# airlift/aircompressor

Hardware: AMD Instinct MI355X
Metric: GiB/s decompressed throughput (Zstd+LZ4) at 1/2/4/8 GPUs; % of HBM3E roofline (higher is better)
Workload: dtype u8; 1 GPU; lz4_decompress, 262144 x 65536 B LZ4 blocks per GPU (BASELINE configs[1]), fragments data ratio=0.50, LZ4 ratio 1.817, batched C-ABI launch, HBM-resident; blocks_per_gpu=262144, block_bytes=65536, distinct_blocks=4096, parallelism=block-sharded x1, no collective, decoder=rings (chosen on the device: 0 of 16384 16-block groups mixed), twopass_fallback_blocks=-1

## Files before the change

### aircompressor_amd/csrc/achip_rings.h

```cpp
#pragma once
#include "achip_device.h"

namespace achip {


template <int GS, int IN_RING, int OUT_RING, int GPL = 1, int PHASED = 0>
struct Rings {
    static constexpr int CHUNK = GS * 16 * GPL;
    static constexpr int LDS_REACH = OUT_RING - CHUNK - 16;
    static_assert((IN_RING & (IN_RING - 1)) == 0 && (OUT_RING & (OUT_RING - 1)) == 0, "rings are powers of two");
    static_assert(IN_RING >= 2 * CHUNK && OUT_RING >= 4 * CHUNK, "ring too small for the chunk size");
    static_assert(!PHASED || (IN_RING >= 4 * CHUNK && GS == 4 && GPL == 1), "the phased form keeps two chunks of input ahead");
    static constexpr bool PH_REFILL = PHASED != 0, PH_FLUSH = false;

    uint8_t* inRing;
    uint8_t* outRing;
    const uint8_t* inAligned;
    uint8_t* outAligned;
    int32_t inBase, outBase;
    int32_t inEndV;
    int32_t inLoadedV;
    int32_t flushedV;
    u32x4 pending[GPL];
    int g;
    uint8_t* stage;

    static constexpr bool UNIFIED = GS == 4 && GPL == 1;

#if !defined(__HIPCC__) && defined(HOSTEMU_RINGS_LOCKSTEP)
    __device__ __forceinline__ void order() const { if (GS > 1) hostemu::group_sync(GS, __FILE__, __LINE__); }
    __device__ __forceinline__ void enter() const { if (GS > 1) hostemu::group_sync(GS, __FILE__, __LINE__); }
#elif !defined(__HIPCC__) && defined(HOSTEMU_RINGS_ORDER_ONLY)
    __device__ __forceinline__ void order() const { if (GS > 1) hostemu::group_sync(GS, __FILE__, __LINE__); }
    __device__ __forceinline__ void enter() const {}
#else
    __device__ __forceinline__ void order() const { wave_mem_order(); }
    __device__ __forceinline__ void enter() const {}
#endif

    __device__ __forceinline__ void init(uint8_t* ldsIn, uint8_t* ldsOut, const uint8_t* in, int32_t inLimit, uint8_t* out, int lane, uint8_t* ldsStage = nullptr)
    {
        inRing = ldsIn;
        outRing = ldsOut;
        stage = ldsStage;
        inBase = (int32_t)((uintptr_t)in & 15);
        outBase = (int32_t)((uintptr_t)out & 15);
        inAligned = in - inBase;
        outAligned = out - outBase;
        inEndV = inLimit + inBase;
        inLoadedV = 0;
        flushedV = 0;
        g = lane;
        if (PHASED) {
            request_pending(16 * g);
        }
        else {
#pragma unroll
            for (int q = 0; q < GPL; q++) {
                pending[q] = fetch_granule(16 * (g + GS * q));
            }
        }
    }

    __device__ __forceinline__ void request_pending(int32_t v) { pending[0] = fetch_granule(v); }
    __device__ __forceinline__ u32x4 take_pending(int32_t) { return pending[0]; }

    __device__ __forceinline__ void reset_input(const uint8_t* in, int32_t inLimit)
    {
        enter();
        inBase = (int32_t)((uintptr_t)in & 15);
        inAligned = in - inBase;
        inEndV = inLimit + inBase;
        inLoadedV = 0;
        order();
#pragma unroll
        for (int q = 0; q < GPL; q++) {
            pending[q] = fetch_granule(16 * (g + GS * q));
        }
    }

    __device__ __forceinline__ u32x4 fetch_granule(int32_t v) const
    {
        u32x4 d = {0, 0, 0, 0};
        if (v >= inBase && v + 16 <= inEndV) {
            d = ld16_global(inAligned + v);
        }
        else if (v + 16 > inBase && v < inEndV) {
            uint32_t w[4] = {0, 0, 0, 0};
#pragma unroll 1
            for (int i = 0; i < 16; i++) {
                const int32_t p = v + i;
                if (p >= inBase && p < inEndV) {
                    w[i >> 2] |= (uint32_t)inAligned[p] << (8 * (i & 3));
                }
            }
            d = u32x4{w[0], w[1], w[2], w[3]};
        }
        return d;
    }

    __device__ __forceinline__ void refill()
    {
        if (PHASED) {
            const int32_t v = inLoadedV + 16 * g;
            *(u32x4*)(inRing + (v & (IN_RING - 1))) = take_pending(v);
            request_pending(v + CHUNK);
            inLoadedV += CHUNK;
            return;
        }
#pragma unroll
        for (int q = 0; q < GPL; q++) {
            const int32_t v = inLoadedV + 16 * (g + GS * q);
            *(u32x4*)(inRing + (v & (IN_RING - 1))) = pending[q];
            pending[q] = fetch_granule(v + CHUNK);
        }
        inLoadedV += CHUNK;
    }
    __device__ __forceinline__ void ensure_input(int32_t pos, int32_t need)
    {
        enter();
        const int32_t want = pos + inBase + need;
        if (want > inLoadedV && inLoadedV < inEndV) {
            do {
                refill();
            } while (want > inLoadedV && inLoadedV < inEndV);
        }
        order();
    }
    __device__ __forceinline__ uint32_t in_u8(int32_t pos) const { return inRing[(pos + inBase) & (IN_RING - 1)]; }

    __device__ __forceinline__ void memory_phase(int32_t ip, int32_t op)
    {
        if (PHASED) {
            enter();
            if (PH_REFILL && inLoadedV - (ip + inBase) <= IN_RING - CHUNK && inLoadedV < inEndV) {
                refill();
            }
            order();
            if (PH_FLUSH) {
                flush_complete(op);
            }
        }
    }

    template <int RING>
    static __device__ __forceinline__ uint32_t ring_ld4(const uint8_t* ring, int32_t pv)
    {
        const int32_t a = pv & ~3;
        const uint32_t lo = *(const uint32_t*)(ring + (a & (RING - 1)));
        const uint32_t hi = *(const uint32_t*)(ring + ((a + 4) & (RING - 1)));
        return alignbyte_u32(hi, lo, (uint32_t)(pv & 3));
    }


    template <int SRC_RING>
    __device__ __forceinline__ void copy_dwords(const uint8_t* src, int32_t sV, int32_t dV, int32_t c)
    {
        copy_dwords_rt(src, SRC_RING - 1, sV, dV, c);
    }

    __device__ __forceinline__ void put4(int32_t dV, uint32_t w, int32_t cnt)
    {
        if (cnt > 0) outRing[dV & (OUT_RING - 1)] = (uint8_t)w;
        if (cnt > 1) outRing[(dV + 1) & (OUT_RING - 1)] = (uint8_t)(w >> 8);
        if (cnt > 2) outRing[(dV + 2) & (OUT_RING - 1)] = (uint8_t)(w >> 16);
        if (cnt > 3) outRing[(dV + 3) & (OUT_RING - 1)] = (uint8_t)(w >> 24);
    }
    template <int SRC_RING>
    __device__ __forceinline__ void copy_small(const uint8_t* src, int32_t sV, int32_t dV, int32_t n)
    {
        const uint32_t w = ring_ld4<SRC_RING>(src, sV + 4 * g);
        enter();
        put4(dV + 4 * g, w, n - 4 * g);
    }

    static __device__ __forceinline__ uint32_t ring_ld4_rt(const uint8_t* ring, int32_t mask, int32_t pv)
    {
        const int32_t a = pv & ~3;
        const uint32_t lo = *(const uint32_t*)(ring + (a & mask));
        const uint32_t hi = *(const uint32_t*)(ring + ((a + 4) & mask));
        return alignbyte_u32(hi, lo, (uint32_t)(pv & 3));
    }
    __device__ __forceinline__ void copy_dwords_rt(const uint8_t* src, int32_t mask, int32_t sV, int32_t dV, int32_t c)
    {
        int32_t head = (4 - (dV & 3)) & 3;
        head = head < c ? head : c;
        constexpr int ITER = CHUNK / (4 * GS);
        uint32_t w[ITER];
#pragma unroll
        for (int q = 0; q < ITER; q++) {
            w[q] = ring_ld4_rt(src, mask, sV + head + 4 * (g + GS * q));
        }
        uint32_t hb[3] = {0, 0, 0};
#pragma unroll
        for (int k = 0; k < 3; k++) {
            if ((k & (GS - 1)) == g && k < head) {
                hb[k] = src[(sV + k) & mask];
            }
        }
        enter();
#pragma unroll
        for (int q = 0; q < ITER; q++) {
            *(uint32_t*)(outRing + ((dV + head + 4 * (g + GS * q)) & (OUT_RING - 1))) = w[q];
        }
#pragma unroll
        for (int k = 0; k < 3; k++) {
            if ((k & (GS - 1)) == g && k < head) {
                outRing[(dV + k) & (OUT_RING - 1)] = (uint8_t)hb[k];
            }
        }
    }

    __device__ __forceinline__ void out_put(int32_t pos, uint32_t byte) { outRing[(pos + outBase) & (OUT_RING - 1)] = (uint8_t)byte; }
    __device__ __forceinline__ uint32_t out_get(int32_t pos) const { return outRing[(pos + outBase) & (OUT_RING - 1)]; }

    __device__ __forceinline__ void flush_complete(int32_t op)
    {
        enter();
        const int32_t opV = op + outBase;
        order();
        while (flushedV + CHUNK <= opV) {
#pragma unroll
            for (int q = 0; q < GPL; q++) {
                const int32_t v = flushedV + 16 * (g + GS * q);
                if (v >= outBase) {
                    *(u32x4*)(outAligned + v) = *(const u32x4*)(outRing + (v & (OUT_RING - 1)));
                }
                else if (v + 16 > outBase) {
                    for (int32_t p = outBase; p < v + 16; p++) {
                        outAligned[p] = outRing[p & (OUT_RING - 1)];
                    }
                }
            }
            flushedV += CHUNK;
        }
        order();
    }
    __device__ __forceinline__ void flush_all(int32_t op)
    {
        flush_complete(op);
        const int32_t opV = op + outBase;
#pragma unroll
        for (int q = 0; q < GPL; q++) {
            const int32_t v = flushedV + 16 * (g + GS * q);
            if (v < opV) {
                if (v >= outBase && v + 16 <= opV) {
                    *(u32x4*)(outAligned + v) = *(const u32x4*)(outRing + (v & (OUT_RING - 1)));
                }
                else {
                    const int32_t lo = v > outBase ? v : outBase;
                    const int32_t hi = v + 16 < opV ? v + 16 : opV;
                    for (int32_t p = lo; p < hi; p++) {
                        outAligned[p] = outRing[p & (OUT_RING - 1)];
                    }
                }
            }
        }
        flushedV = opV & ~15;
        order();
    }

    __device__ __forceinline__ void fill(int32_t op, uint32_t value, int32_t n)
    {
        enter();
        while (n > 0) {
            const int32_t c = n < CHUNK ? n : CHUNK;
            for (int32_t k = g; k < c; k += GS) {
                out_put(op + k, value);
            }
            op += c;
            n -= c;
            flush_complete(op);
        }
    }

    __device__ __forceinline__ void copy_literals(int32_t ip, int32_t op, int32_t n)
    {
        enter();
        if (UNIFIED && n > 4 * GS) {
            while (n > 0) {
                const int32_t c = n < CHUNK ? n : CHUNK;
                ensure_input(ip, c);
                copy_dwords<IN_RING>(inRing, ip + inBase, op + outBase, c);
                ip += c;
                op += c;
                n -= c;
                if (!PH_FLUSH || n > 0) {
                    flush_complete(op);
                }
            }
            return;
        }
        if (n <= 4 * GS) {
            ensure_input(ip, n);
            copy_small<IN_RING>(inRing, ip + inBase, op + outBase, n);
            if (!PH_FLUSH) {
                flush_complete(op + n);
            }
            return;
        }
        while (n > 0) {
            const int32_t c = n < CHUNK ? n : CHUNK;
            ensure_input(ip, c);
            if (c <= (GS > 4 ? GS : 4)) {
                for (int32_t k = g; k < c; k += GS) {
                    out_put(op + k, in_u8(ip + k));
                }
            }
            else {
                copy_dwords<IN_RING>(inRing, ip + inBase, op + outBase, c);
            }
            ip += c;
            op += c;
            n -= c;
            flush_complete(op);
        }
    }

    __device__ __forceinline__ void copy_match(int32_t op, int32_t offset, int32_t n)
    {
        enter();
        if (UNIFIED && !(n <= 4 * GS && offset >= n)) {
            if (stage != nullptr) {
                int32_t dist = offset;
                while (n > 0) {
                    int32_t c = n < CHUNK ? n : CHUNK;
                    c = c < dist ? c : dist;
                    order();
                    if (dist <= LDS_REACH) {
                        copy_dwords<OUT_RING>(outRing, op + outBase - dist, op + outBase, c);
                    }
                    else {
                        if (PH_FLUSH && op + outBase - dist + CHUNK > flushedV) {
                            flush_complete(op);
                            order();
                        }
                        *(u32x4*)(stage + 16 * g) = ld16(outAligned + outBase + (op - dist) + 16 * g);
                        order();
                        copy_dwords<CHUNK>(stage, 0, op + outBase, c);
                    }
                    op += c;
                    n -= c;
                    if (dist < CHUNK) {
                        dist += dist;
                    }
                    if (!PH_FLUSH || n > 0) {
                        flush_complete(op);
                    }
                }
                return;
            }
        }
        if (n <= 4 * GS && offset >= n) {
            order();
            if (offset <= LDS_REACH) {
                copy_small<OUT_RING>(outRing, op + outBase - offset, op + outBase, n);
            }
            else {
                if (PH_FLUSH && op + outBase - offset + 4 * GS > flushedV) {
                    flush_complete(op);
                    order();
                }
                put4(op + outBase + 4 * g, ld4(outAligned + outBase + (op - offset) + 4 * g), n - 4 * g);
            }
            if (!PH_FLUSH) {
                flush_complete(op + n);
            }
            return;
        }
        int32_t c0 = op;
        while (n > 0) {
            const int32_t c = n < CHUNK ? n : CHUNK;
            order();
            if (offset <= LDS_REACH) {
                if (offset >= c && c <= (GS > 4 ? GS : 4)) {
                    for (int32_t j = g; j < c; j += GS) {
                        out_put(c0 + j, out_get(c0 - offset + j));
                    }
                }
                else if (offset >= c) {
                    copy_dwords<OUT_RING>(outRing, c0 + outBase - offset, c0 + outBase, c);
                }
                else {
                    const uint32_t inv = offset == 1 ? 0u : (0xFFFFFFFFu / (uint32_t)offset + 1u);
                    for (int32_t j = g; j < c; j += GS) {
                        const uint32_t q = offset == 1 ? (uint32_t)j : __umulhi((uint32_t)j, inv);
                        out_put(c0 + j, out_get(c0 - offset + (j - (int32_t)q * offset)));
                    }
                }
            }
            else {
                const uint8_t* src = outAligned + outBase + (c0 - offset);
                if (c <= (GS > 4 ? GS : 4)) {
                    for (int32_t j = g; j < c; j += GS) {
                        out_put(c0 + j, src[j]);
                    }
                }
                else {
                    const int32_t dV = c0 + outBase;
                    const int32_t head = (4 - (dV & 3)) & 3;
                    const int32_t nd = (c - head) >> 2;
                    const int32_t t0 = head + 4 * nd;
                    for (int32_t k = g; k < head; k += GS) {
                        outRing[(dV + k) & (OUT_RING - 1)] = src[k];
                    }
                    for (int32_t j = g; j < nd; j += GS) {
                        *(uint32_t*)(outRing + ((dV + head + 4 * j) & (OUT_RING - 1))) = ld4(src + head + 4 * j);
                    }
                    for (int32_t k = t0 + g; k < c; k += GS) {
                        outRing[(dV + k) & (OUT_RING - 1)] = src[k];
                    }
                }
            }
            c0 += c;
            n -= c;
            flush_complete(c0);
        }
    }
};

}
```

### aircompressor_amd/csrc/lz4_decode_body.h

```cpp
#pragma once
#include "achip_rings.h"

namespace achip {

template <int GS, int IN_RING, int OUT_RING, int GPL, int PHASED = 0>
__device__ __forceinline__ void lz4_block_decode(Rings<GS, IN_RING, OUT_RING, GPL, PHASED>& R, const uint8_t* __restrict__ in, int32_t inLimit, int32_t outLimit, int32_t& stOut,
                                                 int32_t& eoOut, int32_t& opOut)
{
    int32_t st = 0;
    int32_t eo = 0;
    int32_t ip = 0;
    int32_t op = 0;

#define LZ4_FAIL(detail, off)                          \
    {                                                  \
        st = mk_status(ACHIP_CLASS_MALFORMED, detail); \
        eo = (int32_t)(off);                           \
        break;                                         \
    }

    if (inLimit == 0) {
        st = mk_status(ACHIP_CLASS_MALFORMED, ACHIP_D_LZ4_INPUT_EMPTY);
    }
    else if (outLimit == 0) {
        if (!(inLimit == 1 && in[0] == 0)) {
            st = mk_status(ACHIP_CLASS_OUTPUT_TOO_SMALL, ACHIP_D_LZ4_EMPTY_OUTPUT);
        }
    }
    else {
        const int32_t fastOutLimit = outLimit - 8;
        R.ensure_input(ip, 4);
        uint32_t t4 = R.template ring_ld4<IN_RING>(R.inRing, ip + R.inBase);
        while (ip < inLimit) {
            const int32_t token = (int32_t)(t4 & 0xFF);
            ip++;

            int32_t lit = token >> 4;
            if (lit == 0xF) {
                if (ip >= inLimit) LZ4_FAIL(ACHIP_D_LZ4_MALFORMED, ip);
                int32_t v = (int32_t)((t4 >> 8) & 0xFF);
                ip++;
                lit = (int32_t)((uint32_t)lit + (uint32_t)v);
                while (v == 255 && ip < inLimit - 15) {
                    R.ensure_input(ip, 1);
                    v = (int32_t)R.in_u8(ip++);
                    lit = (int32_t)((uint32_t)lit + (uint32_t)v);
                }
            }
            if (lit < 0) LZ4_FAIL(ACHIP_D_LZ4_MALFORMED, ip);

            const int64_t litEnd = (int64_t)ip + lit;
            const int64_t litOutLimit = (int64_t)op + lit;
            if (litOutLimit > fastOutLimit - 4 || litEnd > inLimit - 8) {
                if (litOutLimit > outLimit) LZ4_FAIL(ACHIP_D_LZ4_LAST_LITERAL_OUTSIDE, ip);
                if (litEnd != inLimit) LZ4_FAIL(ACHIP_D_LZ4_INPUT_NOT_CONSUMED, ip);
                R.copy_literals(ip, op, lit);
                op += lit;
                break;
            }

            uint32_t o4 = 0;
            const bool early = lit + 3 <= Rings<GS, IN_RING, OUT_RING, GPL, PHASED>::CHUNK;
            if (early) {
                R.ensure_input(ip, lit + 3);
                o4 = R.template ring_ld4<IN_RING>(R.inRing, (int32_t)litEnd + R.inBase);
            }
            R.copy_literals(ip, op, lit);
            op += lit;
            ip = (int32_t)litEnd;
            R.memory_phase(ip, op);

            if (!early) {
                R.ensure_input(ip, 3);
                o4 = R.template ring_ld4<IN_RING>(R.inRing, ip + R.inBase);
            }
            const int32_t offset = (int32_t)(o4 & 0xFFFF);
            ip += 2;
            if (offset == 0 || offset > op) LZ4_FAIL(ACHIP_D_LZ4_OFFSET_OUTSIDE, ip);

            int32_t ml = token & 0xF;
            if (ml == 0xF) {
                if (ip > inLimit - 5) LZ4_FAIL(ACHIP_D_LZ4_MALFORMED, ip);
                int32_t v = (int32_t)((o4 >> 16) & 0xFF);
                ip++;
                ml = (int32_t)((uint32_t)ml + (uint32_t)v);
                bool bad = false;
                while (v == 255) {
                    if (ip > inLimit - 5) {
                        bad = true;
                        break;
                    }
                    R.ensure_input(ip, 1);
                    v = (int32_t)R.in_u8(ip++);
                    ml = (int32_t)((uint32_t)ml + (uint32_t)v);
                }
                if (bad) LZ4_FAIL(ACHIP_D_LZ4_MALFORMED, ip);
            }
            ml = (int32_t)((uint32_t)ml + 4u);
            if (ml < 0) LZ4_FAIL(ACHIP_D_LZ4_MALFORMED, ip);

            const int64_t matchOutLimit = (int64_t)op + ml;
            if (matchOutLimit > fastOutLimit - 4 && matchOutLimit > outLimit - 5) {
                LZ4_FAIL(ACHIP_D_LZ4_LAST_5_LITERALS, ip);
            }
            R.ensure_input(ip, 4);
            t4 = R.template ring_ld4<IN_RING>(R.inRing, ip + R.inBase);
            R.copy_match(op, offset, ml);
            op = (int32_t)matchOutLimit;
        }
        R.flush_all(op);
    }
#undef LZ4_FAIL
    stOut = st;
    eoOut = eo;
    opOut = op;
}

}
```

Before: 2012 GiB/s.

## Streamline 4-lane ring copies with dword-aligned moves and single-step flushes

In the unified decoder path, copy_dwords_rt is replaced by a fixed four-dword-per-lane move aligned to the destination. It merges the partial head dword with the existing ring contents and caps each move at CHUNK minus the misalignment. The flush loop becomes a single-step flush per move, and literals already in the input ring skip the ensure_input check. LZ4 bounds checks in the narrow configuration use precomputed unsigned thresholds. The aim is to cut per-sequence branching and loop overhead. The cost is that correctness now depends on the cap and flush-step invariants, such as flushing at most one chunk per move.

```diff
diff --git a/aircompressor_amd/csrc/achip_rings.h b/aircompressor_amd/csrc/achip_rings.h
--- a/aircompressor_amd/csrc/achip_rings.h
+++ b/aircompressor_amd/csrc/achip_rings.h
@@ -153,6 +153,8 @@
     }
 
 
+    static __device__ __forceinline__ int32_t move_cap(int32_t dV) { return UNIFIED ? CHUNK - (dV & 3) : CHUNK; }
+
     template <int SRC_RING>
     __device__ __forceinline__ void copy_dwords(const uint8_t* src, int32_t sV, int32_t dV, int32_t c)
     {
@@ -183,6 +185,25 @@
     }
     __device__ __forceinline__ void copy_dwords_rt(const uint8_t* src, int32_t mask, int32_t sV, int32_t dV, int32_t c)
     {
+        if (UNIFIED) {
+            const int32_t k = dV & 3;
+            const int32_t s0 = sV - k + 4 * g;
+            const int32_t dI = dV - k + 4 * g;
+            uint32_t w[4];
+#pragma unroll
+            for (int q = 0; q < 4; q++) {
+                w[q] = ring_ld4_rt(src, mask, s0 + 16 * q);
+            }
+            const uint32_t prev = *(const uint32_t*)(outRing + (dI & (OUT_RING - 1)));
+            const uint32_t mine = 0xFFFFFFFFu << (8 * (g == 0 ? k : 0));
+            w[0] = (w[0] & mine) | (prev & ~mine);
+            enter();
+#pragma unroll
+            for (int q = 0; q < 4; q++) {
+                *(uint32_t*)(outRing + ((dI + 16 * q) & (OUT_RING - 1))) = w[q];
+            }
+            return;
+        }
         int32_t head = (4 - (dV & 3)) & 3;
         head = head < c ? head : c;
         constexpr int ITER = CHUNK / (4 * GS);
@@ -230,6 +251,29 @@
                     for (int32_t p = outBase; p < v + 16; p++) {
                         outAligned[p] = outRing[p & (OUT_RING - 1)];
                     }
+                }
+            }
+            flushedV += CHUNK;
+        }
+        order();
+    }
+    __device__ __forceinline__ void flush_step(int32_t op)
+    {
+        if (!UNIFIED) {
+            flush_complete(op);
+            return;
+        }
+        enter();
+        const int32_t opV = op + outBase;
+        order();
+        if (flushedV + CHUNK <= opV) {
+            const int32_t v = flushedV + 16 * g;
+            if (flushedV != 0 || v >= outBase) {
+                *(u32x4*)(outAligned + v) = *(const u32x4*)(outRing + (v & (OUT_RING - 1)));
+            }
+            else if (v + 16 > outBase) {
+                for (int32_t p = outBase; p < v + 16; p++) {
+                    outAligned[p] = outRing[p & (OUT_RING - 1)];
                 }
             }
             flushedV += CHUNK;
@@ -279,14 +323,15 @@
         enter();
         if (UNIFIED && n > 4 * GS) {
             while (n > 0) {
-                const int32_t c = n < CHUNK ? n : CHUNK;
+                const int32_t cap = move_cap(op + outBase);
+                const int32_t c = n < cap ? n : cap;
                 ensure_input(ip, c);
                 copy_dwords<IN_RING>(inRing, ip + inBase, op + outBase, c);
                 ip += c;
                 op += c;
                 n -= c;
                 if (!PH_FLUSH || n > 0) {
-                    flush_complete(op);
+                    flush_step(op);
                 }
             }
             return;
@@ -295,7 +340,7 @@
             ensure_input(ip, n);
             copy_small<IN_RING>(inRing, ip + inBase, op + outBase, n);
             if (!PH_FLUSH) {
-                flush_complete(op + n);
+                flush_step(op + n);
             }
             return;
         }
@@ -317,6 +362,24 @@
         }
     }
 
+    __device__ __forceinline__ void copy_literals_resident(int32_t ip, int32_t op, int32_t n)
+    {
+        static_assert(UNIFIED && !PH_FLUSH, "the 4-lane decoders only");
+        enter();
+        if (n <= 4 * GS) {
+            copy_small<IN_RING>(inRing, ip + inBase, op + outBase, n);
+            flush_step(op + n);
+            return;
+        }
+        const int32_t cap = move_cap(op + outBase);
+        const int32_t c = n < cap ? n : cap;
+        copy_dwords<IN_RING>(inRing, ip + inBase, op + outBase, c);
+        flush_step(op + c);
+        if (n > c) {
+            copy_literals(ip + c, op + c, n - c);
+        }
+    }
+
     __device__ __forceinline__ void copy_match(int32_t op, int32_t offset, int32_t n)
     {
         enter();
@@ -324,7 +387,8 @@
             if (stage != nullptr) {
                 int32_t dist = offset;
                 while (n > 0) {
-                    int32_t c = n < CHUNK ? n : CHUNK;
+                    const int32_t cap = move_cap(op + outBase);
+                    int32_t c = n < cap ? n : cap;
                     c = c < dist ? c : dist;
                     order();
                     if (dist <= LDS_REACH) {
@@ -341,11 +405,11 @@
                     }
                     op += c;
                     n -= c;
-                    if (dist < CHUNK) {
+                    if (dist < CHUNK && c == dist) {
                         dist += dist;
                     }
                     if (!PH_FLUSH || n > 0) {
-                        flush_complete(op);
+                        flush_step(op);
                     }
                 }
                 return;
@@ -364,13 +428,17 @@
                 put4(op + outBase + 4 * g, ld4(outAligned + outBase + (op - offset) + 4 * g), n - 4 * g);
             }
             if (!PH_FLUSH) {
-                flush_complete(op + n);
+                flush_step(op + n);
             }
             return;
         }
         int32_t c0 = op;
         while (n > 0) {
-            const int32_t c = n < CHUNK ? n : CHUNK;
+            int32_t c = n < CHUNK ? n : CHUNK;
+            if (UNIFIED) {
+                const int32_t cap = move_cap(c0 + outBase);
+                c = c < cap ? c : cap;
+            }
             order();
             if (offset <= LDS_REACH) {
                 if (offset >= c && c <= (GS > 4 ? GS : 4)) {
diff --git a/aircompressor_amd/csrc/lz4_decode_body.h b/aircompressor_amd/csrc/lz4_decode_body.h
--- a/aircompressor_amd/csrc/lz4_decode_body.h
+++ b/aircompressor_amd/csrc/lz4_decode_body.h
@@ -29,6 +29,10 @@
     }
     else {
         const int32_t fastOutLimit = outLimit - 8;
+        constexpr bool NARROW = GS == 4 && GPL == 1;
+        const uint32_t litOutFast = (uint32_t)(outLimit - 11 > 0 ? outLimit - 11 : 0);
+        const uint32_t litEndFast = (uint32_t)(inLimit - 7 > 0 ? inLimit - 7 : 0);
+        const uint32_t matchOutBad = (uint32_t)(outLimit - 4 > 0 ? outLimit - 4 : 0);
         R.ensure_input(ip, 4);
         uint32_t t4 = R.template ring_ld4<IN_RING>(R.inRing, ip + R.inBase);
         while (ip < inLimit) {
@@ -51,7 +55,8 @@
 
             const int64_t litEnd = (int64_t)ip + lit;
             const int64_t litOutLimit = (int64_t)op + lit;
-            if (litOutLimit > fastOutLimit - 4 || litEnd > inLimit - 8) {
+            const uint32_t litEndN = (uint32_t)ip + (uint32_t)lit, litOutN = (uint32_t)op + (uint32_t)lit;
+            if (NARROW ? (litOutN >= litOutFast || litEndN >= litEndFast) : (litOutLimit > fastOutLimit - 4 || litEnd > inLimit - 8)) {
                 if (litOutLimit > outLimit) LZ4_FAIL(ACHIP_D_LZ4_LAST_LITERAL_OUTSIDE, ip);
                 if (litEnd != inLimit) LZ4_FAIL(ACHIP_D_LZ4_INPUT_NOT_CONSUMED, ip);
                 R.copy_literals(ip, op, lit);
@@ -65,7 +70,17 @@
                 R.ensure_input(ip, lit + 3);
                 o4 = R.template ring_ld4<IN_RING>(R.inRing, (int32_t)litEnd + R.inBase);
             }
-            R.copy_literals(ip, op, lit);
+            if constexpr (NARROW) {
+                if (early) {
+                    R.copy_literals_resident(ip, op, lit);
+                }
+                else {
+                    R.copy_literals(ip, op, lit);
+                }
+            }
+            else {
+                R.copy_literals(ip, op, lit);
+            }
             op += lit;
             ip = (int32_t)litEnd;
             R.memory_phase(ip, op);
@@ -100,7 +115,7 @@
             if (ml < 0) LZ4_FAIL(ACHIP_D_LZ4_MALFORMED, ip);
 
             const int64_t matchOutLimit = (int64_t)op + ml;
-            if (matchOutLimit > fastOutLimit - 4 && matchOutLimit > outLimit - 5) {
+            if (NARROW ? (uint32_t)op + (uint32_t)ml >= matchOutBad : (matchOutLimit > fastOutLimit - 4 && matchOutLimit > outLimit - 5)) {
                 LZ4_FAIL(ACHIP_D_LZ4_LAST_5_LITERALS, ip);
             }
             R.ensure_input(ip, 4);
```

Measured after the change: 1974 GiB/s. -1.9%, worse.

## Track prefetched input granule position and defer literal flush in phased rings

Applied to the files above, without the earlier changes.

In the phased ring decoder, the prefetched input granule now records which position it belongs to (pendingV). Refill paths that jump ahead fetch directly, and the memory phase consumes the prefetch only when it matches. Long literal runs keep their own one-chunk-ahead fetch, the last literal flush is deferred until after the memory phase, and byte-wise edge handling is moved into noinline helpers to cut register pressure and code size. The aim is to overlap global loads with decoding and reduce wasted or stalled fetches, at the cost of extra bookkeeping and some redundant refetches when positions mismatch.

```diff
diff --git a/aircompressor_amd/csrc/achip_rings.h b/aircompressor_amd/csrc/achip_rings.h
--- a/aircompressor_amd/csrc/achip_rings.h
+++ b/aircompressor_amd/csrc/achip_rings.h
@@ -3,6 +3,24 @@
 
 namespace achip {
 
+
+__device__ __attribute__((noinline)) inline u32x4 ring_fetch_edge(const uint8_t* p, int32_t lo, int32_t hi)
+{
+    uint32_t w[4] = {0, 0, 0, 0};
+#pragma unroll 1
+    for (int i = lo; i < hi; i++) {
+        w[i >> 2] |= (uint32_t)p[i] << (8 * (i & 3));
+    }
+    return u32x4{w[0], w[1], w[2], w[3]};
+}
+__device__ __attribute__((noinline)) inline void ring_store_edge(uint8_t* p, u32x4 d, int32_t lo, int32_t hi)
+{
+    const uint32_t w[4] = {d.x, d.y, d.z, d.w};
+#pragma unroll 1
+    for (int i = lo; i < hi; i++) {
+        p[i] = (uint8_t)(w[i >> 2] >> (8 * (i & 3)));
+    }
+}
 
 template <int GS, int IN_RING, int OUT_RING, int GPL = 1, int PHASED = 0>
 struct Rings {
@@ -11,6 +29,7 @@
     static_assert((IN_RING & (IN_RING - 1)) == 0 && (OUT_RING & (OUT_RING - 1)) == 0, "rings are powers of two");
     static_assert(IN_RING >= 2 * CHUNK && OUT_RING >= 4 * CHUNK, "ring too small for the chunk size");
     static_assert(!PHASED || (IN_RING >= 4 * CHUNK && GS == 4 && GPL == 1), "the phased form keeps two chunks of input ahead");
+    static constexpr bool OUTLINE_EDGES = PHASED != 0;
     static constexpr bool PH_REFILL = PHASED != 0, PH_FLUSH = false;
 
     uint8_t* inRing;
@@ -22,6 +41,7 @@
     int32_t inLoadedV;
     int32_t flushedV;
     u32x4 pending[GPL];
+    int32_t pendingV;
     int g;
     uint8_t* stage;
 
@@ -52,7 +72,8 @@
         flushedV = 0;
         g = lane;
         if (PHASED) {
-            request_pending(16 * g);
+            pendingV = CHUNK;
+            pending[0] = fetch_granule(CHUNK + 16 * g);
         }
         else {
 #pragma unroll
@@ -62,8 +83,6 @@
         }
     }
 
-    __device__ __forceinline__ void request_pending(int32_t v) { pending[0] = fetch_granule(v); }
-    __device__ __forceinline__ u32x4 take_pending(int32_t) { return pending[0]; }
 
     __device__ __forceinline__ void reset_input(const uint8_t* in, int32_t inLimit)
     {
@@ -86,15 +105,20 @@
             d = ld16_global(inAligned + v);
         }
         else if (v + 16 > inBase && v < inEndV) {
-            uint32_t w[4] = {0, 0, 0, 0};
+            if (OUTLINE_EDGES) {
+                d = ring_fetch_edge(inAligned + v, v < inBase ? inBase - v : 0, v + 16 > inEndV ? inEndV - v : 16);
+            }
+            else {
+                uint32_t w[4] = {0, 0, 0, 0};
 #pragma unroll 1
-            for (int i = 0; i < 16; i++) {
-                const int32_t p = v + i;
-                if (p >= inBase && p < inEndV) {
-                    w[i >> 2] |= (uint32_t)inAligned[p] << (8 * (i & 3));
-                }
-            }
-            d = u32x4{w[0], w[1], w[2], w[3]};
+                for (int i = 0; i < 16; i++) {
+                    const int32_t p = v + i;
+                    if (p >= inBase && p < inEndV) {
+                        w[i >> 2] |= (uint32_t)inAligned[p] << (8 * (i & 3));
+                    }
+                }
+                d = u32x4{w[0], w[1], w[2], w[3]};
+            }
         }
         return d;
     }
@@ -103,8 +127,7 @@
     {
         if (PHASED) {
             const int32_t v = inLoadedV + 16 * g;
-            *(u32x4*)(inRing + (v & (IN_RING - 1))) = take_pending(v);
-            request_pending(v + CHUNK);
+            *(u32x4*)(inRing + (v & (IN_RING - 1))) = fetch_granule(v);
             inLoadedV += CHUNK;
             return;
         }
@@ -134,7 +157,15 @@
         if (PHASED) {
             enter();
             if (PH_REFILL && inLoadedV - (ip + inBase) <= IN_RING - CHUNK && inLoadedV < inEndV) {
-                refill();
+                const int32_t v = inLoadedV + 16 * g;
+                u32x4 d = pending[0];
+                if (pendingV != inLoadedV) {
+                    d = fetch_granule(v);
+                }
+                *(u32x4*)(inRing + (v & (IN_RING - 1))) = d;
+                inLoadedV += CHUNK;
+                pending[0] = fetch_granule(v + CHUNK);
+                pendingV = inLoadedV;
             }
             order();
             if (PH_FLUSH) {
@@ -227,8 +258,13 @@
                     *(u32x4*)(outAligned + v) = *(const u32x4*)(outRing + (v & (OUT_RING - 1)));
                 }
                 else if (v + 16 > outBase) {
-                    for (int32_t p = outBase; p < v + 16; p++) {
-                        outAligned[p] = outRing[p & (OUT_RING - 1)];
+                    if (OUTLINE_EDGES) {
+                        ring_store_edge(outAligned + v, *(const u32x4*)(outRing + (v & (OUT_RING - 1))), outBase - v, 16);
+                    }
+                    else {
+                        for (int32_t p = outBase; p < v + 16; p++) {
+                            outAligned[p] = outRing[p & (OUT_RING - 1)];
+                        }
                     }
                 }
             }
@@ -250,8 +286,13 @@
                 else {
                     const int32_t lo = v > outBase ? v : outBase;
                     const int32_t hi = v + 16 < opV ? v + 16 : opV;
-                    for (int32_t p = lo; p < hi; p++) {
-                        outAligned[p] = outRing[p & (OUT_RING - 1)];
+                    if (OUTLINE_EDGES) {
+                        ring_store_edge(outAligned + v, *(const u32x4*)(outRing + (v & (OUT_RING - 1))), lo - v, hi - v);
+                    }
+                    else {
+                        for (int32_t p = lo; p < hi; p++) {
+                            outAligned[p] = outRing[p & (OUT_RING - 1)];
+                        }
                     }
                 }
             }
@@ -274,18 +315,39 @@
         }
     }
 
+    template <bool DEFER_LAST = false>
     __device__ __forceinline__ void copy_literals(int32_t ip, int32_t op, int32_t n)
     {
         enter();
         if (UNIFIED && n > 4 * GS) {
+            const bool longRun = PHASED && n > CHUNK;
+            u32x4 ahead = {0, 0, 0, 0};
+            if (longRun) {
+                ahead = fetch_granule(inLoadedV + 16 * g);
+            }
             while (n > 0) {
                 const int32_t c = n < CHUNK ? n : CHUNK;
-                ensure_input(ip, c);
+                if (longRun) {
+                    enter();
+                    const int32_t want = ip + inBase + c;
+                    if (want > inLoadedV && inLoadedV < inEndV) {
+                        do {
+                            const int32_t v = inLoadedV + 16 * g;
+                            *(u32x4*)(inRing + (v & (IN_RING - 1))) = ahead;
+                            inLoadedV += CHUNK;
+                            ahead = fetch_granule(v + CHUNK);
+                        } while (want > inLoadedV && inLoadedV < inEndV);
+                    }
+                    order();
+                }
+                else {
+                    ensure_input(ip, c);
+                }
                 copy_dwords<IN_RING>(inRing, ip + inBase, op + outBase, c);
                 ip += c;
                 op += c;
                 n -= c;
-                if (!PH_FLUSH || n > 0) {
+                if (!(PH_FLUSH || DEFER_LAST) || n > 0) {
                     flush_complete(op);
                 }
             }
@@ -294,11 +356,12 @@
         if (n <= 4 * GS) {
             ensure_input(ip, n);
             copy_small<IN_RING>(inRing, ip + inBase, op + outBase, n);
-            if (!PH_FLUSH) {
+            if (!(PH_FLUSH || DEFER_LAST)) {
                 flush_complete(op + n);
             }
             return;
         }
+        static_assert(!DEFER_LAST || UNIFIED, "deferred literal flushes: the unified copies only");
         while (n > 0) {
             const int32_t c = n < CHUNK ? n : CHUNK;
             ensure_input(ip, c);
diff --git a/aircompressor_amd/csrc/lz4_decode_body.h b/aircompressor_amd/csrc/lz4_decode_body.h
--- a/aircompressor_amd/csrc/lz4_decode_body.h
+++ b/aircompressor_amd/csrc/lz4_decode_body.h
@@ -65,10 +65,13 @@
                 R.ensure_input(ip, lit + 3);
                 o4 = R.template ring_ld4<IN_RING>(R.inRing, (int32_t)litEnd + R.inBase);
             }
-            R.copy_literals(ip, op, lit);
+            R.template copy_literals<PHASED != 0>(ip, op, lit);
             op += lit;
             ip = (int32_t)litEnd;
             R.memory_phase(ip, op);
+            if (PHASED) {
+                R.flush_complete(op);
+            }
 
             if (!early) {
                 R.ensure_input(ip, 3);
```

Result: slower. 1932 GiB/s before, 1573 GiB/s after (-18.6%).
